# guodashun/peg-in-hole-gym

Measured on AMD Instinct MI355X. Metric: env-steps/sec, higher is better.
Workload: dtype f32

## Files before the change

### peg_in_hole_gym_amd/csrc/pih_common.h

```cpp
#pragma once
#include <string.h>
#include "../../include/pih.h"
#include "../../include/pih_model.h"
#include "pih_math.h"

namespace pih {

constexpr int NL = PIH_NL, ANL = PIH_ARM_NL, ONL = PIH_OBJ_NL, ND = PIH_NDOF;
constexpr int NSAMP = PIH_PIPE_NSAMP;
constexpr int CMAX = 48;
constexpr int CAMAX = 12;
constexpr int CL = 20;
constexpr int NROWC = 3 * CMAX;
constexpr int WPS = 39;
constexpr int WMS = 31;
constexpr int NMOT = 32;
constexpr int NLIM = 18;
static_assert(PIH_DBG_UDOT + ND <= PIH_DBG_NCONTACT && PIH_DBG_CONTACT + PIH_DBG_CONTACT_STRIDE * CMAX <= PIH_DBG_DINV &&
              PIH_DBG_DINV + 3 * CMAX <= PIH_DBG_CYCLES && PIH_DBG_XCC_ID < PIH_DEBUG_WORDS, "debug words of the peg-in-hole step (include/pih.h PIH_DBG_*) overlap");

PIH_CONST int L_PARENT[NL] = PIH_LINK_PARENT;
PIH_CONST int L_JTYPE[NL] = PIH_LINK_JTYPE;
PIH_CONST real L_RFIX[NL][9] = PIH_LINK_RFIX;
PIH_CONST real L_TFIX[NL][3] = PIH_LINK_TFIX;
// ... 422 lines not shown
    real tip[7]; tip_pose_serial(S, tip);
    Q4 tornq; tornq.x = tip[3]; tornq.y = tip[4]; tornq.z = tip[5]; tornq.w = tip[6];
    V3 rv = mul(q_to_m(tornq), mk(0, S[PIH_S_RANDY], 0));
    V3 tpos = mk(tip[0], tip[1], tip[2]) + rv;
    V3 tp = vel_constraint(eep, tpos, P.dv);
    if (st == 2 && st_prev != 2) o.grasp_angle = (real)atan2(rv.y, rv.x);
    if (st == 4 && st_prev != 4) o.attach_qz = tip[5];
    real yaw = yaw_from_quat(tornq);
    V3 hole = ld3(HOLE_POS);
    Q4 tq; tq.x = 0; tq.y = 0; tq.z = 0; tq.w = 1;
    int do_ik = 0;
    if (st == 1) { tp.z += (real)0.05; tq = quat_from_euler(0, -PIH_PI, PIH_PI / 2 + yaw); do_ik = 1; }
    else if (st == 2) { tp.z -= (real)0.01; tq = quat_from_euler(0, -PIH_PI, PIH_PI / 2 + yaw); do_ik = 1; }
    else if (st == 4) { tp = vel_constraint(eep, hole - mk((real)0.2, 0, 0), P.dv); tq = quat_from_euler(0, -PIH_PI, -PIH_PI); do_ik = 1; }
    else if (st == 5) { tp = vel_constraint(eep, hole - mk((real)0.04, 0, 0), P.dv); tq = quat_from_euler(0, -PIH_PI, -PIH_PI); do_ik = 1; }
    else if (st == 6) { tp = hole; tq = quat_from_euler(0, -PIH_PI, -PIH_PI); do_ik = 1; }
    else if (st == 8) { tp = mk((real)0.2, (real)-0.6, (real)0.4); tq = quat_from_euler(0, -PIH_PI, PIH_PI / 2); do_ik = 1; }
    if (do_ik) {
      real qs[7];
      ik_chain<PandaChain>(sw, ikT, P, q, tp, tq, qs);
#pragma unroll
      for (int i = 0; i < 7; i++) o.target[i] = qs[i];
    }
    const bool closed = st >= 3 && st < 7;
    const real ft = closed ? (real)0.006 : (real)0.02;
    o.target[7] = ft; o.target[8] = ft;
  }
  return o;
}
PIH_HD void controller_targets(real* S, const Params& P, const real* action) { const CtrlOut o = controller_compute(S, P, action); controller_apply(S, o); }

template <class W> PIH_HD void controller_rows(W& w, Shared& sh, const Params& P, int part = 0) {
  real* S = sh.S;
  int posctl_arm = 0; real kp_arm = 0, imp_arm = 1, kp_f = 0, imp_f = 1; int posctl_f = 0;
  if (P.mode == 0) {
    posctl_arm = posctl_f = 1; kp_arm = kp_f = 1; imp_arm = imp_f = (real)100000.0 * P.dt;
  } else {
    const int st = (int)S[PIH_S_FSM];
    if (st == 9) S[PIH_S_DONE] = 1;
    if (st >= 1) { posctl_arm = 1; kp_arm = (real)0.1; imp_arm = (real)(5.0 * 240.0) * P.dt; }
    const bool closed = st >= 3 && st < 7;
    posctl_f = 1; kp_f = (real)0.1; imp_f = (closed ? (real)20000 : (real)20) * P.dt;
  }
  w.par(NMOT, [&](int m) {
    if ((part == 1 && m < 9) || (part == 2 && m >= 9)) return;
    real vt = 0, imp = 1;
    if (m < 7) { if (posctl_arm) { vt = kp_arm * (S[PIH_S_TARGET + m] - S[PIH_S_QARM + m]) / P.dt; imp = imp_arm; } }
    else if (m < 9) { if (posctl_f) { vt = kp_f * (S[PIH_S_TARGET + m] - S[PIH_S_QARM + m]) / P.dt; imp = imp_f; } }
    sh.mrec[m][MR_RHS] = part == 2 ? (vt - sh.u[m]) * sh.mrec[m][MR_DINV] : vt;
    sh.mrec[m][MR_IMP] = imp;
  });
}

template <class W> PIH_HD void collide(W& w, Shared& sh, const Params& P) {
  const real r = (real)PIH_PIPE_RADIUS, margin = P.margin;
  w.par(NSAMP, [&](int i) {
    int L = ANL + SAMP_LINK[i];
    V3 p = ld3(sh.LO[L]) + mul(ldm(sh.a.LR[L]), mk(0, SAMP_Y[i], 0));
    st3(sh.a.SP[i], p);
  });
  auto emit = [&](int slot, int la, int lb, int key, V3 p, V3 n, real depth, real mu) {
    sh.c_la[slot] = la; sh.c_lb[slot] = lb; sh.c_key[slot] = key; st3(sh.c_p[slot], p); st3(sh.c_n[slot], n);
    sh.c_depth[slot] = depth; sh.c_mu[slot] = clampr(mu, -PIH_MAX_FRICTION, PIH_MAX_FRICTION);
  };
  w.alloc_reset(0);
  w.par_all(NSAMP, [&](int i, bool in) {
    bool valid = false; V3 sp = mk(0, 0, 0); real depth = 0; int L = 0;
    if (in && SAMP_VERTEX[i]) {
      sp = ld3(sh.a.SP[i]); depth = sp.z - (real)PIH_TABLE_Z - r; L = ANL + SAMP_LINK[i];
      valid = depth < margin;
    }
    int slot = w.alloc(valid);
    if (valid && slot < CMAX) {
      int vi = 0;
      { int s = SAMP_LINK[i]; vi = SAMP_Y[i] > (real)0.02 && s == 23 ? 24 : s; }
      emit(slot, L, -1, vi, mk(sp.x, sp.y, sp.z - r - (real)0.5 * depth), mk(0, 0, 1), depth, L_MU[L] * (real)PIH_TABLE_MU);
    }
  });
  const real hl = (real)PIH_HOLE_HALFLEN, rcx = (real)(0.5 * (PIH_HOLE_RIN + PIH_HOLE_ROUT)), hw = (real)(0.5 * (PIH_HOLE_ROUT - PIH_HOLE_RIN));
  w.par_all(NSAMP, [&](int i, bool in) {
    bool valid = false; V3 n = mk(0, 0, 0), p = mk(0, 0, 0); real depth = 0; int L = 0;
    if (in) {
      V3 sp = ld3(sh.a.SP[i]); V3 d = sp - ld3(HOLE_POS);
      real a = d.x, rho = (real)sqrt(d.y * d.y + d.z * d.z);
      real dx = absr(a) - hl, dy = absr(rho - rcx) - hw;
      if (!(dx > r + margin || dy > r + margin)) {
        real sa = a >= 0 ? (real)1 : (real)-1, sr = rho >= rcx ? (real)1 : (real)-1, ga, gr, sdf;
        if (dx <= 0 && dy <= 0) { if (dx > dy) { ga = sa; gr = 0; sdf = dx; } else { ga = 0; gr = sr; sdf = dy; } }
        else { real mx = dx > 0 ? dx : 0, my = dy > 0 ? dy : 0; sdf = (real)sqrt(mx * mx + my * my); ga = sa * mx / sdf; gr = sr * my / sdf; }
        depth = sdf - r;
        if (depth < margin && rho > (real)1e-9) {
          V3 rh = mk(0, d.y / rho, d.z / rho);
          n = mk(ga, gr * rh.y, gr * rh.z); p = sp - (r + (real)0.5 * depth) * n; L = ANL + SAMP_LINK[i]; valid = true;
        }
      }
    }
    int slot = w.alloc(valid);
    if (valid && slot < CMAX) emit(slot, L, -1, 100 + i, p, n, depth, L_MU[L] * (real)PIH_HOLE_MU);
  });
  int nca = 0;
  {
    const bool attached = P.mode == 1 && sh.S[PIH_S_FSM] >= 4 && sh.S[PIH_S_FSM] <= 6;
    const int before = w.alloc_count();
    w.par_all(1, [&](int i, bool in) {
      bool valid = in && i == 0 && attached;
      int slot = w.alloc(valid);
      if (valid && slot < CMAX) {
        int g = (int)sh.S[PIH_S_GRASP];
        int L = g == 0 ? ANL : NL - 1;
        V3 a1 = ld3(sh.LO[L]) + mul(ldm(sh.a.LR[L]), mk(0, (g == 0 ? (real)0.045 : (real)0.015) + sh.S[PIH_S_RANDY], 0));
        V3 ee; M3 eR; ee_pose(sh, ee, eR);
        V3 d = a1 - ee; real dist = norm(d);
        V3 n = dist > (real)1e-9 ? ((real)1 / dist) * d : mk(1, 0, 0);
        emit(slot, L, PIH_EE_PARENT, 2000, (real)0.5 * (a1 + ee), n, dist, (real)-1);
      }
    });
    w.par_all(1, [&](int i, bool in) {
      bool valid = in && i == 0 && attached && !P.attachball;
      int slot = w.alloc(valid);
      if (valid && slot < CMAX) {
        int g = (int)sh.S[PIH_S_GRASP];
        int L = g == 0 ? ANL : NL - 1;
        V3 ee; M3 eR; ee_pose(sh, ee, eR);
        const M3 Rcf = q_to_m(quat_from_euler(0, -PIH_PI, PIH_PI / 2 + sh.S[PIH_S_ATTACH_QZ]));
        const M3 Rc = mul(ldm(sh.a.LR[L]), Rcf);
        M3 eRt; for (int r = 0; r < 3; r++) for (int c = 0; c < 3; c++) eRt.m[3 * r + c] = eR.m[3 * c + r];
        const Q4 qe = m_to_q(mul(Rc, eRt));
        const V3 xyz = mk(qe.x, qe.y, qe.z);
        const real sn = norm(xyz); real ang = 2 * (real)atan2(sn, qe.w);
        if (ang > PIH_PI) ang -= 2 * PIH_PI;
        const V3 th = sn > (real)1e-12 ? (ang / sn) * xyz : mk(0, 0, 0);
        emit(slot, L, PIH_EE_PARENT, 2001, th, mk(1, 0, 0), 0, (real)-2);
      }
    });
    nca += w.alloc_count() - before;
  }
  if (P.armcol) w.par(PIH_ARM_NSPH, [&](int i) { const int L = ASPH_LINK[i]; st3(sh.a.ASP[i], ld3(sh.LO[L]) + mul(ldm(sh.a.LR[L]), ld3(ASPH_C[i]))); });
  if (P.armcol & 1) {
    const int before = w.alloc_count();
    const int allowed = CAMAX - nca;
    w.par_all(PIH_ARM_NSPH, [&](int i, bool in) {
      bool valid = false; V3 cw = mk(0, 0, 0); real depth = 0, rs = 0; int L = 0;
      if (in) {
        L = ASPH_LINK[i]; rs = ASPH_R[i];
        cw = ld3(sh.a.ASP[i]);
        depth = cw.z - (real)PIH_TABLE_Z - rs;
        valid = depth < margin;
      }
      int slot = w.alloc(valid);
      if (valid && slot < CMAX && (slot - before) < allowed) emit(slot, L, -1, 3000 + i, mk(cw.x, cw.y, cw.z - rs - (real)0.5 * depth), mk(0, 0, 1), depth, L_MU[L] * (real)PIH_TABLE_MU);
    });
    int used = w.alloc_count() - before;
    if (used > allowed) { used = allowed; w.alloc_reset(before + allowed); }
    nca += used;
  }
  const real padreach = norm(ld3(FBOX_H)) + r + margin + (real)1e-4;
  for (int f = 0; f < 2; f++) {
    const int LF = PIH_FINGER_LINK0 + f;
    M3 Rf = ldm(sh.a.LR[LF]); V3 bc = ld3(sh.LO[LF]) + mul(Rf, ld3(FBOX_C[f])); V3 bh = ld3(FBOX_H);
    const int before = w.alloc_count();
    const int allowed = CAMAX - nca;
    w.par_all(NSAMP, [&](int i, bool in) {
      bool valid = false; V3 n = mk(0, 0, 0), p = mk(0, 0, 0); real depth = 0; int L = 0;
      if (in) {
        V3 sp = ld3(sh.a.SP[i]); V3 d = sp - bc;
        if (dot(d, d) <= padreach * padreach) {
          V3 pl = tmul(Rf, d);
          V3 q = mk(clampr(pl.x, -bh.x, bh.x), clampr(pl.y, -bh.y, bh.y), clampr(pl.z, -bh.z, bh.z));
          bool inside = q.x == pl.x && q.y == pl.y && q.z == pl.z;
          V3 nl; real sdf;
          if (inside) {
            real bx = bh.x - absr(pl.x), by = bh.y - absr(pl.y), bz = bh.z - absr(pl.z);
            int ax = 0; real best = bx;
            if (by < best) { best = by; ax = 1; }
            if (bz < best) { best = bz; ax = 2; }
            nl = mk(ax == 0 ? (pl.x >= 0 ? (real)1 : (real)-1) : 0, ax == 1 ? (pl.y >= 0 ? (real)1 : (real)-1) : 0, ax == 2 ? (pl.z >= 0 ? (real)1 : (real)-1) : 0);
            sdf = -best;
          } else { V3 df = pl - q; sdf = norm(df); nl = ((real)1 / sdf) * df; }
          depth = sdf - r;
          if (depth < margin) { n = mul(Rf, nl); p = sp - (r + (real)0.5 * depth) * n; L = ANL + SAMP_LINK[i]; valid = true; }
        }
      }
      int slot = w.alloc(valid);
      if (valid && slot < CMAX && (slot - before) < allowed) emit(slot, L, LF, 300 + f * NSAMP + i, p, n, depth, L_MU[L] * L_MU[LF]);
    });
    int used = w.alloc_count() - before;
    if (used > allowed) { used = allowed; w.alloc_reset(before + allowed); }
    nca += used;
  }
  if (P.armcol & 2) {
    const int before = w.alloc_count();
    const int allowed = CAMAX - nca;
    w.par_all(NSAMP, [&](int i, bool in) {
      bool valid = false; V3 n = mk(0, 0, 0), p = mk(0, 0, 0); real depth = margin; int L = 0, bs = 0;
      if (in) {
        const V3 sp = ld3(sh.a.SP[i]);
#pragma unroll
        for (int s = PIH_ARM_PIPE_SPH0; s < PIH_ARM_NSPH; s++) {
          const V3 d = sp - ld3(sh.a.ASP[s]);
          const real d2 = dot(d, d), reach = margin + r + ASPH_R[s];
          if (d2 < reach * reach) {
            const real dist = (real)sqrt(d2), dep = dist - r - ASPH_R[s];
            if (dep < depth && dist > (real)1e-9) { depth = dep; bs = s; n = ((real)1 / dist) * d; valid = true; }
          }
        }
        if (valid) { p = sp - (r + (real)0.5 * depth) * n; L = ANL + SAMP_LINK[i]; }
      }
      int slot = w.alloc(valid);
      if (valid && slot < CMAX && (slot - before) < allowed) emit(slot, L, ASPH_LINK[bs], 5000 + bs * NSAMP + i, p, n, depth, L_MU[L] * L_MU[ASPH_LINK[bs]]);
    });
    int used = w.alloc_count() - before;
    if (used > allowed) { used = allowed; w.alloc_reset(before + allowed); }
    nca += used;
  }
  if (P.selfcol) {
    w.par_all(253, [&](int idx, bool in) {
      bool valid = false; V3 n = mk(0, 0, 0), p = mk(0, 0, 0); real depth = 0; int s = 0, t = 0;
      if (in) {
        s = (int)((real)0.5 * ((real)45 - (real)sqrt((real)(2025 - 8 * idx))));
        if ((s + 1) * (44 - s) / 2 <= idx) s++;
        if (s * (45 - s) / 2 > idx) s--;
        t = s + 2 + idx - s * (45 - s) / 2;
        auto vtx = [&](int v) -> V3 { int si = v == 0 ? 0 : (v == 24 ? NSAMP - 1 : 7 + 5 * (v - 1)); return ld3(sh.a.SP[si]); };
        V3 p1 = vtx(s), q1 = vtx(s + 1), p2 = vtx(t), q2 = vtx(t + 1);
        V3 dm = (p1 + q1) - (p2 + q2);
        V3 d1 = q1 - p1, d2 = q2 - p2;
        real a = dot(d1, d1), e = dot(d2, d2);
        const real reach = (real)sqrt(a) + (real)sqrt(e) + 2 * (2 * r + margin) + (real)1e-4;
        if (dot(dm, dm) <= reach * reach) {
          V3 rr = p1 - p2;
          real f = dot(d2, rr), ss, tt;
          const real EPS = (real)1e-12;
          if (a <= EPS && e <= EPS) { ss = tt = 0; }
          else if (a <= EPS) { ss = 0; tt = clampr(f / e, 0, 1); }
          else {
            real c = dot(d1, rr);
            if (e <= EPS) { tt = 0; ss = clampr(-c / a, 0, 1); }
            else {
              real b = dot(d1, d2), den = a * e - b * b;
              ss = den > EPS ? clampr((b * f - c * e) / den, 0, 1) : (real)0;
              tt = (b * ss + f) / e;
              if (tt < 0) { tt = 0; ss = clampr(-c / a, 0, 1); } else if (tt > 1) { tt = 1; ss = clampr((b - c) / a, 0, 1); }
            }
          }
          V3 c1 = p1 + ss * d1, c2 = p2 + tt * d2, d = c1 - c2;
          real dist = norm(d); depth = dist - 2 * r;
          if (depth < margin && dist >= (real)1e-9) { n = ((real)1 / dist) * d; p = (real)0.5 * (c1 + c2); valid = true; }
        }
      }
      int slot = w.alloc(valid);
      if (valid && slot < CMAX) emit(slot, ANL + s, ANL + t, 1000 + s * 24 + t, p, n, depth, L_MU[ANL + s] * L_MU[ANL + t]);
    });
  }
  int nc = w.alloc_count(); if (nc > CMAX) nc = CMAX;
  sh.nc = nc; sh.nca = nca;
}

PIH_HD void aba_root_inverse(Shared& sh, const real* Mx, areal* rootp) {
  areal Mq[6][6], Iv[6][6];
  for (int i = 0; i < 6; i++) for (int j = 0; j < 6; j++) { Mq[i][j] = Mx[8 * i + j]; Iv[i][j] = i == j ? (areal)1 : (areal)0; }
#pragma unroll
  for (int k = 0; k < 6; k++) {
    areal pv = (areal)1 / Mq[k][k];
#pragma unroll
    for (int j = 0; j < 6; j++) { Mq[k][j] *= pv; Iv[k][j] *= pv; }
#pragma unroll
    for (int i = 0; i < 6; i++) if (i != k) {
      areal f = Mq[i][k];
#pragma unroll
      for (int j = 0; j < 6; j++) { Mq[i][j] -= f * Mq[k][j]; Iv[i][j] -= f * Iv[k][j]; }
    }
  }
  for (int i = 0; i < 6; i++) { for (int j = 0; j < 6; j++) sh.Inv6[6 * i + j] = (real)Iv[i][j]; rootp[i] = Mx[8 * i + 6]; }
}
PIH_HD int aba_own_word(int i, int j) {
  const int ii = i < 3 ? i : i - 3, jj = j < 3 ? j : j - 3;
  const int sym = ii == jj ? ii : ii + jj + 2;
  if (i >= 6 || j >= 7) return 27;
  if (j == 6) return 21 + i;
  if (i < 3 && j < 3) return sym;
  if (i >= 3 && j >= 3) return 15 + sym;
  if (i < 3) return 6 + 3 * i + jj;
  return 6 + 3 * j + ii;
}
static_assert(NROWC >= 144, "scratch of the inward sweep aliases r_lam");

struct RowOut { real* wa; real* wp; };
PIH_HD real response(const Shared& sh, int la, int lb, V3 p, V3 dir, int jm, RowOut out, V3* dvp_out = nullptr, bool ang = false) {
  real jw = 0; V3 dvp = mk(0, 0, 0);
  bool arm = (la >= 0 && la < ANL) || (lb >= 0 && lb < ANL) || (jm >= 0 && jm < ANL);
  bool obj = (la >= ANL) || (lb >= ANL) || (jm >= ANL);
  if (arm && out.wa) {
    const bool aa_ = la >= 0 && la < ANL, ab_ = lb >= 0 && lb < ANL;
    const V3 rA = p - ld3(sh.LO[aa_ ? la : 0]), rB = p - ld3(sh.LO[ab_ ? lb : 0]);
    const V3 tqa = ang ? dir : cross(rA, dir), tqb = ang ? dir : cross(rB, dir), tl = ang ? mk(0, 0, 0) : dir;
    struct LinkC { V3 a, Ua, Ul, r; real Di; };
    auto linkc = [&](int L) __attribute__((always_inline)) -> LinkC {
      LinkC c; c.a = ld3(sh.LA[L]); c.Ua = ld3(sh.AU[L]); c.Ul = ld3(sh.AU[L] + 3); c.r = ld3(sh.AR[L]); c.Di = sh.ADinv[L]; return c;
    };
    V3 Qa[ANL], Ql[ANL]; real uu[ANL];
#pragma unroll
    for (int L = 0; L < ANL; L++) { Qa[L] = mk(0, 0, 0); Ql[L] = mk(0, 0, 0); }
    LinkC nx = linkc(ANL - 1);
#pragma unroll
    for (int L = ANL - 1; L >= 0; L--) {
      const LinkC c = nx;
// ... 204 lines not shown
```

### peg_in_hole_gym_amd/csrc/pih_wave.h

```cpp
#pragma once
#include <type_traits>
#include "pih_common.h"
#include "pih_mailbox.h"

namespace pih {

PIH_HD void debug_store_time(real* dbg, int at, long long t) { dbg[at] = (real)(t & 0xFFFF); dbg[at + 1] = (real)((t >> 16) & 0xFFFF); dbg[at + 2] = (real)((t >> 32) & 0xFFFF); }
PIH_HD void debug_store_hw_id(real* dbg) { dbg[PIH_DBG_HW_ID] = (real)(__builtin_amdgcn_s_getreg((15 << 11) | 4) & 0xFFFF); dbg[PIH_DBG_XCC_ID] = (real)__builtin_amdgcn_s_getreg((3 << 11) | 20); }

struct Wave {
  int l;
  int counter;
  static constexpr bool controller_inline = false;
  real* dbg = nullptr; int dbgmode = 0; long long t0 = 0, t1 = 0;
  PIH_HD void stamp(int k) { if (dbg && dbgmode == 2) { long long t = __builtin_readcyclecounter(); if (l == 0) dbg[PIH_DBG_CYCLES + k] = (real)(t - t0); t0 = t; } }
  PIH_HD void trace(int at, long long t) { if (l != 0) return; debug_store_time(dbg, at, t); if (at == PIH_DBG_T_START) debug_store_hw_id(dbg); }
  PIH_HD void phase_begin() { if (dbg && dbgmode == 2) { t1 = __builtin_readcyclecounter(); trace(PIH_DBG_T_START, (long long)__builtin_amdgcn_s_memrealtime()); } }
  PIH_HD void phase(int k) { if (dbg && dbgmode == 2) { long long t = __builtin_readcyclecounter(); if (l == 0) dbg[PIH_DBG_CYCLES + k] = (real)(t - t1); t1 = t; if (k == 7) trace(PIH_DBG_T_END, (long long)__builtin_amdgcn_s_memrealtime()); } }
  PIH_HD int lane() const { return l; }
  bool prio_on = true;
  PIH_HD void priority(int contacts) {
    if (!prio_on) return;
    if (contacts > 20) __builtin_amdgcn_s_setprio(3);
    else if (contacts > 14) __builtin_amdgcn_s_setprio(2);
// ... 103 lines not shown
#pragma unroll
  for (int off = 1; off < 32; off <<= 1) {
    const int src = vidx - off;
    const int sb = lane_byte((active && src >= cs) ? src : 63);
    M3 Rs; V3 os;
#pragma unroll
    for (int k = 0; k < 9; k++) Rs.m[k] = from_lane(R.m[k], sb);
    os = mk(from_lane(o.x, sb), from_lane(o.y, sb), from_lane(o.z, sb));
    o = os + mul(Rs, o); R = mul(Rs, R);
  }
  if (active) {
    stm(sh.a.LR[L], R); st3(sh.LO[L], o);
    st3(sh.LA[L], mul(R, ld3(L_AXIS[L])));
    st3(sh.a.LRC[L], mul(R, ld3(L_COM[L])));
    sts3(sh.a.LIC[L], rot_sym(R, lds3(L_INERTIA[L])));
  }
  w.sync();
}
PIH_HD V3 from_lane3(V3 v, int byte_addr) { return mk(from_lane(v.x, byte_addr), from_lane(v.y, byte_addr), from_lane(v.z, byte_addr)); }
PIH_HD V3 chain_prefix_sum(V3 t, int lane, int chain_start) {
  V3 acc = t;
#pragma unroll
  for (int off = 1; off < 32; off <<= 1) {
    const int src = lane - off;
    const V3 o = from_lane3(acc, 4 * (src < 0 ? 0 : src));
    if (src >= chain_start) acc = acc + o;
  }
  return acc;
}
PIH_HD void link_velocities_scan(Shared& sh, int lane) {
  const bool active = lane < NL;
  const int L = active ? lane : NL - 1;
  const int jt = L == ANL ? PIH_JT_FLOATING : ((L == ANL - 1 || L == ANL - 2) ? PIH_JT_PRISMATIC : PIH_JT_REVOLUTE);
  const int par = (L == 0 || L == ANL) ? -1 : (L == ANL - 1 ? ANL - 3 : L - 1);
  const int cs = L < ANL ? 0 : ANL, d = link_dof(L);
  const V3 aq = sh.u[d] * ld3(sh.LA[L]);
  const V3 tw = jt == PIH_JT_FLOATING ? ld3(&sh.u[d + 3]) : (jt == PIH_JT_REVOLUTE ? aq : mk(0, 0, 0));
  V3 wv = chain_prefix_sum(tw, lane, cs);
  const V3 tw7 = from_lane3(tw, 4 * (ANL - 2));
  if (L == ANL - 1) wv = wv - tw7;
  const V3 wp = from_lane3(wv, 4 * (par < 0 ? 0 : par));
  V3 tv;
  if (jt == PIH_JT_FLOATING) tv = ld3(&sh.u[d]);
  else {
    tv = jt == PIH_JT_PRISMATIC ? aq : mk(0, 0, 0);
    if (par >= 0) tv = tv + cross(wp, ld3(sh.LO[L]) - ld3(sh.LO[par]));
  }
  V3 vv = chain_prefix_sum(tv, lane, cs);
  const V3 tv7 = from_lane3(tv, 4 * (ANL - 2));
  if (L == ANL - 1) vv = vv - tv7;
  if (active) { st3(sh.VW[L], wv); st3(sh.VV[L], vv); }
}
PIH_HD void link_velocities(Wave& w, Shared& sh) { w.sync(); link_velocities_scan(sh, w.lane()); w.sync(); }

PIH_HD void aba_inward(Wave& w, Shared& sh, areal* rootp) {
  real* const Mx = sh.r_lam;
  {
    const int l = w.lane(), i = l >> 3, j = l & 7;
    const int ia = i < 3 ? i : (i < 6 ? i - 3 : 0), ja = j < 3 ? j : (j < 6 ? j - 3 : 0);
    const int i1 = ia == 2 ? 0 : ia + 1, i2 = ia == 0 ? 2 : ia - 1, j1 = ja == 2 ? 0 : ja + 1, j2 = ja == 0 ? 2 : ja - 1;
    const bool typeA = i < 3 && j < 3, typeB = i < 3 && j >= 3 && j < 6, typeBt = i >= 3 && i < 6 && j < 3, typeP = i < 3 && j == 6;
    const int own_off = aba_own_word(i, j);
    int kA = 0, kB = 0, s1 = l, s2 = l;
    if (typeA) { kA = i1; kB = i2; s1 = 8 * j + 3 + i2; s2 = 8 * j + 3 + i1; }
    else if (typeB) { kA = i1; kB = i2; s1 = 8 * (3 + i2) + j; s2 = 8 * (3 + i1) + j; }
    else if (typeBt) { kA = j1; kB = j2; s1 = 8 * (3 + j2) + i; s2 = 8 * (3 + j1) + i; }
    else if (typeP) { kA = i1; kB = i2; s1 = 8 * (3 + i2) + 6; s2 = 8 * (3 + i1) + 6; }
    const real m1 = (typeA || typeB || typeBt || typeP) ? (real)1 : (real)0, m2 = typeA ? (real)1 : (real)0;
    int s3 = l, s4 = l, s5 = l, s6 = l, s7 = l, s8 = l;
    if (typeA) { s3 = 8 * i + 3 + j1; s4 = 8 * (3 + i2) + 3 + j1; s5 = 8 * (3 + i1) + 3 + j1; s6 = 8 * i + 3 + j2; s7 = 8 * (3 + i2) + 3 + j2; s8 = 8 * (3 + i1) + 3 + j2; }
    const int sUj = j < 6 ? 8 * j : l;
    auto link = [&](int L, real m, bool up) __attribute__((always_inline)) -> real {
      const int jt = joint_type(L);
      const int sb = jt == PIH_JT_REVOLUTE ? 0 : 3;
      const V3 a = ld3(sh.LA[L]);
      const real rA = m1 * sh.AR[L][kA], rB = m1 * sh.AR[L][kB], rG = m2 * sh.AR[L][j2], rK = m2 * sh.AR[L][j1];
      const real cj = j < 6 ? sh.a.CB[L][j] : (real)0;
      const int js = j - sb;
      const real sj = js == 0 ? a.x : (js == 1 ? a.y : (js == 2 ? a.z : (real)0));
      const real Ui = sum8(m * sj);
      const real Uj = from_lane(Ui, 4 * sUj);
      const real D = a.x * rdlane(Ui, 8 * sb) + a.y * rdlane(Ui, 8 * (sb + 1)) + a.z * rdlane(Ui, 8 * (sb + 2));
      const real tau = 0;
      const real u = tau - (a.x * rdlane(m, 8 * sb + 6) + a.y * rdlane(m, 8 * (sb + 1) + 6) + a.z * rdlane(m, 8 * (sb + 2) + 6));
      const real Di = (real)1 / D;
      if (j == 0 && i < 6) sh.AU[L][i] = Ui;
      if (l == 0) { sh.ADinv[L] = Di; sh.Au[L] = u; }
      if (!up) return 0;
      real ma = j < 6 ? m - Ui * Uj * Di : m;
      const real s = sum8(j < 6 ? ma * cj : (real)0);
      if (j == 6) ma = m + s + Ui * (u * Di);
      const real X1 = from_lane(ma, 4 * s1), X2 = from_lane(ma, 4 * s2), X3 = from_lane(ma, 4 * s3), X4 = from_lane(ma, 4 * s4),
                 X5 = from_lane(ma, 4 * s5), X6 = from_lane(ma, 4 * s6), X7 = from_lane(ma, 4 * s7), X8 = from_lane(ma, 4 * s8);
      return ma + rA * X1 - rB * X2 - ((X3 + rA * X4 - rB * X5) * rG - (X6 + rA * X7 - rB * X8) * rK);
    };
    real carry_p = 0, carry_a = 0, hold = 0;
#pragma nounroll
    for (int k = 0; k < 8; k++) {
      const int Lp = NL - 1 - k, La = ANL - 1 - k;
      const real own_p = sh.a.IAP[Lp][own_off], own_a = sh.a.IAP[La][own_off];
      const real mp = k == 0 ? own_p : own_p + carry_p;
      const real ma = k < 2 ? own_a : own_a + carry_a;
      const real vp = link(Lp, mp, true), va = link(La, ma, true);
      carry_p = vp;
      if (k == 0) hold = va;
      else if (k == 1) carry_a = va + hold;
// ... 714 lines not shown
```

Before: 11.99 million.

## Fuse collision narrow-phase into a single-wave pass with register-held candidates

Adds a Wave-specialised collide that computes every sample's table, tube, finger-pad and arm-sphere candidates in one pass, keeping sample points and arm-sphere centres in registers instead of re-reading shared memory per test and synchronising between separate parallel loops. Per-link friction and sphere constants are resolved from constexpr tables by select chains, and inline asm pins keep values in vector or scalar registers. Contact slots are still allocated in the original order so the emitted contacts stay identical. It raises register pressure because many candidates are live at once, which could lower occupancy.

```diff
diff --git a/peg_in_hole_gym_amd/csrc/pih_common.h b/peg_in_hole_gym_amd/csrc/pih_common.h
--- a/peg_in_hole_gym_amd/csrc/pih_common.h
+++ b/peg_in_hole_gym_amd/csrc/pih_common.h
@@ -498,52 +498,159 @@
   });
 }
 
+struct Cand { bool valid; V3 p, n; real depth; };
+PIH_HD Cand no_cand(real depth = 0) { Cand c; c.valid = false; c.p = mk(0, 0, 0); c.n = mk(0, 0, 0); c.depth = depth; return c; }
+PIH_HD V3 sample_point(const Shared& sh, int L, real y) { return ld3(sh.LO[L]) + mul(ldm(sh.a.LR[L]), mk(0, y, 0)); }
+PIH_HD int vertex_key(int slink, real sy) { return sy > (real)0.02 && slink == 23 ? 24 : slink; }
+PIH_HD void emit_contact(Shared& sh, int slot, int la, int lb, int key, V3 p, V3 n, real depth, real mu) {
+  sh.c_la[slot] = la; sh.c_lb[slot] = lb; sh.c_key[slot] = key; st3(sh.c_p[slot], p); st3(sh.c_n[slot], n);
+  sh.c_depth[slot] = depth; sh.c_mu[slot] = clampr(mu, -PIH_MAX_FRICTION, PIH_MAX_FRICTION);
+}
+PIH_HD Cand sphere_vs_table(V3 c, real rs, real margin) {
+  Cand o; o.depth = c.z - (real)PIH_TABLE_Z - rs; o.valid = o.depth < margin;
+  o.p = mk(c.x, c.y, c.z - rs - (real)0.5 * o.depth); o.n = mk(0, 0, 1);
+  return o;
+}
+PIH_HD Cand sample_vs_tube(V3 sp, V3 hole, real r, real margin) {
+  const real hl = (real)PIH_HOLE_HALFLEN, rcx = (real)(0.5 * (PIH_HOLE_RIN + PIH_HOLE_ROUT)), hw = (real)(0.5 * (PIH_HOLE_ROUT - PIH_HOLE_RIN));
+  Cand o = no_cand();
+  V3 d = sp - hole;
+  real a = d.x, rho = (real)sqrt(d.y * d.y + d.z * d.z);
+  real dx = absr(a) - hl, dy = absr(rho - rcx) - hw;
+  if (!(dx > r + margin || dy > r + margin)) {
+    real sa = a >= 0 ? (real)1 : (real)-1, sr = rho >= rcx ? (real)1 : (real)-1, ga, gr, sdf;
+    if (dx <= 0 && dy <= 0) { if (dx > dy) { ga = sa; gr = 0; sdf = dx; } else { ga = 0; gr = sr; sdf = dy; } }
+    else { real mx = dx > 0 ? dx : 0, my = dy > 0 ? dy : 0; sdf = (real)sqrt(mx * mx + my * my); ga = sa * mx / sdf; gr = sr * my / sdf; }
+    o.depth = sdf - r;
+    if (o.depth < margin && rho > (real)1e-9) {
+      V3 rh = mk(0, d.y / rho, d.z / rho);
+      o.n = mk(ga, gr * rh.y, gr * rh.z); o.p = sp - (r + (real)0.5 * o.depth) * o.n; o.valid = true;
+    }
+  }
+  return o;
+}
+PIH_HD real pad_reach(V3 bh, real r, real margin) { return norm(bh) + r + margin + (real)1e-4; }
+PIH_HD Cand sample_vs_pad(V3 sp, const M3& Rf, V3 bc, V3 bh, real padreach, real r, real margin) {
+  Cand o = no_cand();
+  V3 d = sp - bc;
+  if (dot(d, d) <= padreach * padreach) {
+    V3 pl = tmul(Rf, d);
+    V3 q = mk(clampr(pl.x, -bh.x, bh.x), clampr(pl.y, -bh.y, bh.y), clampr(pl.z, -bh.z, bh.z));
+    bool inside = q.x == pl.x && q.y == pl.y && q.z == pl.z;
+    V3 nl; real sdf;
+    if (inside) {
+      real bx = bh.x - absr(pl.x), by = bh.y - absr(pl.y), bz = bh.z - absr(pl.z);
+      int ax = 0; real best = bx;
+      if (by < best) { best = by; ax = 1; }
+      if (bz < best) { best = bz; ax = 2; }
+      nl = mk(ax == 0 ? (pl.x >= 0 ? (real)1 : (real)-1) : 0, ax == 1 ? (pl.y >= 0 ? (real)1 : (real)-1) : 0, ax == 2 ? (pl.z >= 0 ? (real)1 : (real)-1) : 0);
+      sdf = -best;
+    } else { V3 df = pl - q; sdf = norm(df); nl = ((real)1 / sdf) * df; }
+    o.depth = sdf - r;
+    if (o.depth < margin) { o.n = mul(Rf, nl); o.p = sp - (r + (real)0.5 * o.depth) * o.n; o.valid = true; }
+  }
+  return o;
+}
+template <class FC, class FR> PIH_HD Cand sample_vs_arm_spheres(V3 sp, FC centre, FR radius, real r, real margin, int& bs) {
+  Cand o = no_cand(margin);
+  bs = 0;
+#pragma unroll
+  for (int s = PIH_ARM_PIPE_SPH0; s < PIH_ARM_NSPH; s++) {
+    const V3 d = sp - centre(s);
+    const real d2 = dot(d, d), reach = margin + r + radius(s);
+    if (d2 < reach * reach) {
+      const real dist = (real)sqrt(d2), dep = dist - r - radius(s);
+      if (dep < o.depth && dist > (real)1e-9) { o.depth = dep; bs = s; o.n = ((real)1 / dist) * d; o.valid = true; }
+    }
+  }
+  if (o.valid) o.p = sp - (r + (real)0.5 * o.depth) * o.n;
+  return o;
+}
+PIH_HD void pair_of_index(int idx, int& s, int& t) {
+  s = (int)((real)0.5 * ((real)45 - (real)sqrt((real)(2025 - 8 * idx))));
+  if ((s + 1) * (44 - s) / 2 <= idx) s++;
+  if (s * (45 - s) / 2 > idx) s--;
+  t = s + 2 + idx - s * (45 - s) / 2;
+}
+PIH_HD int vertex_sample(int v) { return v == 0 ? 0 : (v == 24 ? NSAMP - 1 : 7 + 5 * (v - 1)); }
+PIH_HD Cand segment_pair(V3 p1, V3 q1, V3 p2, V3 q2, real r, real margin) {
+  Cand o = no_cand();
+  V3 dm = (p1 + q1) - (p2 + q2);
+  V3 d1 = q1 - p1, d2 = q2 - p2;
+  real a = dot(d1, d1), e = dot(d2, d2);
+  const real reach = (real)sqrt(a) + (real)sqrt(e) + 2 * (2 * r + margin) + (real)1e-4;
+  if (dot(dm, dm) <= reach * reach) {
+    V3 rr = p1 - p2;
+    real f = dot(d2, rr), ss, tt;
+    const real EPS = (real)1e-12;
+    if (a <= EPS && e <= EPS) { ss = tt = 0; }
+    else if (a <= EPS) { ss = 0; tt = clampr(f / e, 0, 1); }
+    else {
+      real c = dot(d1, rr);
+      if (e <= EPS) { tt = 0; ss = clampr(-c / a, 0, 1); }
+      else {
+        real b = dot(d1, d2), den = a * e - b * b;
+        ss = den > EPS ? clampr((b * f - c * e) / den, 0, 1) : (real)0;
+        tt = (b * ss + f) / e;
+        if (tt < 0) { tt = 0; ss = clampr(-c / a, 0, 1); } else if (tt > 1) { tt = 1; ss = clampr((b - c) / a, 0, 1); }
+      }
+    }
+    V3 c1 = p1 + ss * d1, c2 = p2 + tt * d2, d = c1 - c2;
+    real dist = norm(d); o.depth = dist - 2 * r;
+    if (o.depth < margin && dist >= (real)1e-9) { o.n = ((real)1 / dist) * d; o.p = (real)0.5 * (c1 + c2); o.valid = true; }
+  }
+  return o;
+}
+PIH_HD Cand attach_ball_contact(Shared& sh, int& L) {
+  Cand o;
+  int g = (int)sh.S[PIH_S_GRASP];
+  L = g == 0 ? ANL : NL - 1;
+  V3 a1 = ld3(sh.LO[L]) + mul(ldm(sh.a.LR[L]), mk(0, (g == 0 ? (real)0.045 : (real)0.015) + sh.S[PIH_S_RANDY], 0));
+  V3 ee; M3 eR; ee_pose(sh, ee, eR);
+  V3 d = a1 - ee; real dist = norm(d);
+  o.n = dist > (real)1e-9 ? ((real)1 / dist) * d : mk(1, 0, 0);
+  o.p = (real)0.5 * (a1 + ee); o.depth = dist; o.valid = true;
+  return o;
+}
+PIH_HD Cand attach_weld_contact(Shared& sh, int& L) {
+  Cand o;
+  int g = (int)sh.S[PIH_S_GRASP];
+  L = g == 0 ? ANL : NL - 1;
+  V3 ee; M3 eR; ee_pose(sh, ee, eR);
+  const M3 Rcf = q_to_m(quat_from_euler(0, -PIH_PI, PIH_PI / 2 + sh.S[PIH_S_ATTACH_QZ]));
+  const M3 Rc = mul(ldm(sh.a.LR[L]), Rcf);
+  M3 eRt; for (int r = 0; r < 3; r++) for (int c = 0; c < 3; c++) eRt.m[3 * r + c] = eR.m[3 * c + r];
+  const Q4 qe = m_to_q(mul(Rc, eRt));
+  const V3 xyz = mk(qe.x, qe.y, qe.z);
+  const real sn = norm(xyz); real ang = 2 * (real)atan2(sn, qe.w);
+  if (ang > PIH_PI) ang -= 2 * PIH_PI;
+  o.p = sn > (real)1e-12 ? (ang / sn) * xyz : mk(0, 0, 0);
+  o.n = mk(1, 0, 0); o.depth = 0; o.valid = true;
+  return o;
+}
+
 template <class W> PIH_HD void collide(W& w, Shared& sh, const Params& P) {
   const real r = (real)PIH_PIPE_RADIUS, margin = P.margin;
-  w.par(NSAMP, [&](int i) {
-    int L = ANL + SAMP_LINK[i];
-    V3 p = ld3(sh.LO[L]) + mul(ldm(sh.a.LR[L]), mk(0, SAMP_Y[i], 0));
-    st3(sh.a.SP[i], p);
-  });
-  auto emit = [&](int slot, int la, int lb, int key, V3 p, V3 n, real depth, real mu) {
-    sh.c_la[slot] = la; sh.c_lb[slot] = lb; sh.c_key[slot] = key; st3(sh.c_p[slot], p); st3(sh.c_n[slot], n);
-    sh.c_depth[slot] = depth; sh.c_mu[slot] = clampr(mu, -PIH_MAX_FRICTION, PIH_MAX_FRICTION);
-  };
+  w.stamp(16);
+  w.par(NSAMP, [&](int i) { st3(sh.a.SP[i], sample_point(sh, ANL + SAMP_LINK[i], SAMP_Y[i])); });
+  auto emit = [&](int slot, int la, int lb, int key, V3 p, V3 n, real depth, real mu) { emit_contact(sh, slot, la, lb, key, p, n, depth, mu); };
   w.alloc_reset(0);
   w.par_all(NSAMP, [&](int i, bool in) {
-    bool valid = false; V3 sp = mk(0, 0, 0); real depth = 0; int L = 0;
-    if (in && SAMP_VERTEX[i]) {
-      sp = ld3(sh.a.SP[i]); depth = sp.z - (real)PIH_TABLE_Z - r; L = ANL + SAMP_LINK[i];
-      valid = depth < margin;
-    }
-    int slot = w.alloc(valid);
-    if (valid && slot < CMAX) {
-      int vi = 0;
-      { int s = SAMP_LINK[i]; vi = SAMP_Y[i] > (real)0.02 && s == 23 ? 24 : s; }
-      emit(slot, L, -1, vi, mk(sp.x, sp.y, sp.z - r - (real)0.5 * depth), mk(0, 0, 1), depth, L_MU[L] * (real)PIH_TABLE_MU);
+    Cand c = no_cand();
+    if (in && SAMP_VERTEX[i]) c = sphere_vs_table(ld3(sh.a.SP[i]), r, margin);
+    int slot = w.alloc(c.valid);
+    if (c.valid && slot < CMAX) {
+      const int L = ANL + SAMP_LINK[i];
+      emit(slot, L, -1, vertex_key(SAMP_LINK[i], SAMP_Y[i]), c.p, c.n, c.depth, L_MU[L] * (real)PIH_TABLE_MU);
     }
   });
-  const real hl = (real)PIH_HOLE_HALFLEN, rcx = (real)(0.5 * (PIH_HOLE_RIN + PIH_HOLE_ROUT)), hw = (real)(0.5 * (PIH_HOLE_ROUT - PIH_HOLE_RIN));
   w.par_all(NSAMP, [&](int i, bool in) {
-    bool valid = false; V3 n = mk(0, 0, 0), p = mk(0, 0, 0); real depth = 0; int L = 0;
-    if (in) {
-      V3 sp = ld3(sh.a.SP[i]); V3 d = sp - ld3(HOLE_POS);
-      real a = d.x, rho = (real)sqrt(d.y * d.y + d.z * d.z);
-      real dx = absr(a) - hl, dy = absr(rho - rcx) - hw;
-      if (!(dx > r + margin || dy > r + margin)) {
-        real sa = a >= 0 ? (real)1 : (real)-1, sr = rho >= rcx ? (real)1 : (real)-1, ga, gr, sdf;
-        if (dx <= 0 && dy <= 0) { if (dx > dy) { ga = sa; gr = 0; sdf = dx; } else { ga = 0; gr = sr; sdf = dy; } }
-        else { real mx = dx > 0 ? dx : 0, my = dy > 0 ? dy : 0; sdf = (real)sqrt(mx * mx + my * my); ga = sa * mx / sdf; gr = sr * my / sdf; }
-        depth = sdf - r;
-        if (depth < margin && rho > (real)1e-9) {
-          V3 rh = mk(0, d.y / rho, d.z / rho);
-          n = mk(ga, gr * rh.y, gr * rh.z); p = sp - (r + (real)0.5 * depth) * n; L = ANL + SAMP_LINK[i]; valid = true;
-        }
-      }
-    }
-    int slot = w.alloc(valid);
-    if (valid && slot < CMAX) emit(slot, L, -1, 100 + i, p, n, depth, L_MU[L] * (real)PIH_HOLE_MU);
+    Cand c = no_cand();
+    if (in) c = sample_vs_tube(ld3(sh.a.SP[i]), ld3(HOLE_POS), r, margin);
+    int slot = w.alloc(c.valid);
+    if (c.valid && slot < CMAX) { const int L = ANL + SAMP_LINK[i]; emit(slot, L, -1, 100 + i, c.p, c.n, c.depth, L_MU[L] * (real)PIH_HOLE_MU); }
   });
+  w.stamp(17);
   int nca = 0;
   {
     const bool attached = P.mode == 1 && sh.S[PIH_S_FSM] >= 4 && sh.S[PIH_S_FSM] <= 6;
@@ -551,33 +658,12 @@
     w.par_all(1, [&](int i, bool in) {
       bool valid = in && i == 0 && attached;
       int slot = w.alloc(valid);
-      if (valid && slot < CMAX) {
-        int g = (int)sh.S[PIH_S_GRASP];
-        int L = g == 0 ? ANL : NL - 1;
-        V3 a1 = ld3(sh.LO[L]) + mul(ldm(sh.a.LR[L]), mk(0, (g == 0 ? (real)0.045 : (real)0.015) + sh.S[PIH_S_RANDY], 0));
-        V3 ee; M3 eR; ee_pose(sh, ee, eR);
-        V3 d = a1 - ee; real dist = norm(d);
-        V3 n = dist > (real)1e-9 ? ((real)1 / dist) * d : mk(1, 0, 0);
-        emit(slot, L, PIH_EE_PARENT, 2000, (real)0.5 * (a1 + ee), n, dist, (real)-1);
-      }
+      if (valid && slot < CMAX) { int L; const Cand c = attach_ball_contact(sh, L); emit(slot, L, PIH_EE_PARENT, 2000, c.p, c.n, c.depth, (real)-1); }
     });
     w.par_all(1, [&](int i, bool in) {
       bool valid = in && i == 0 && attached && !P.attachball;
       int slot = w.alloc(valid);
-      if (valid && slot < CMAX) {
-        int g = (int)sh.S[PIH_S_GRASP];
-        int L = g == 0 ? ANL : NL - 1;
-        V3 ee; M3 eR; ee_pose(sh, ee, eR);
-        const M3 Rcf = q_to_m(quat_from_euler(0, -PIH_PI, PIH_PI / 2 + sh.S[PIH_S_ATTACH_QZ]));
-        const M3 Rc = mul(ldm(sh.a.LR[L]), Rcf);
-        M3 eRt; for (int r = 0; r < 3; r++) for (int c = 0; c < 3; c++) eRt.m[3 * r + c] = eR.m[3 * c + r];
-        const Q4 qe = m_to_q(mul(Rc, eRt));
-        const V3 xyz = mk(qe.x, qe.y, qe.z);
-        const real sn = norm(xyz); real ang = 2 * (real)atan2(sn, qe.w);
-        if (ang > PIH_PI) ang -= 2 * PIH_PI;
-        const V3 th = sn > (real)1e-12 ? (ang / sn) * xyz : mk(0, 0, 0);
-        emit(slot, L, PIH_EE_PARENT, 2001, th, mk(1, 0, 0), 0, (real)-2);
-      }
+      if (valid && slot < CMAX) { int L; const Cand c = attach_weld_contact(sh, L); emit(slot, L, PIH_EE_PARENT, 2001, c.p, c.n, c.depth, (real)-2); }
     });
     nca += w.alloc_count() - before;
   }
@@ -586,118 +672,63 @@
     const int before = w.alloc_count();
     const int allowed = CAMAX - nca;
     w.par_all(PIH_ARM_NSPH, [&](int i, bool in) {
-      bool valid = false; V3 cw = mk(0, 0, 0); real depth = 0, rs = 0; int L = 0;
-      if (in) {
-        L = ASPH_LINK[i]; rs = ASPH_R[i];
-        cw = ld3(sh.a.ASP[i]);
-        depth = cw.z - (real)PIH_TABLE_Z - rs;
-        valid = depth < margin;
-      }
-      int slot = w.alloc(valid);
-      if (valid && slot < CMAX && (slot - before) < allowed) emit(slot, L, -1, 3000 + i, mk(cw.x, cw.y, cw.z - rs - (real)0.5 * depth), mk(0, 0, 1), depth, L_MU[L] * (real)PIH_TABLE_MU);
+      Cand c = no_cand();
+      if (in) c = sphere_vs_table(ld3(sh.a.ASP[i]), ASPH_R[i], margin);
+      int slot = w.alloc(c.valid);
+      if (c.valid && slot < CMAX && (slot - before) < allowed) { const int L = ASPH_LINK[i]; emit(slot, L, -1, 3000 + i, c.p, c.n, c.depth, L_MU[L] * (real)PIH_TABLE_MU); }
     });
     int used = w.alloc_count() - before;
     if (used > allowed) { used = allowed; w.alloc_reset(before + allowed); }
     nca += used;
   }
-  const real padreach = norm(ld3(FBOX_H)) + r + margin + (real)1e-4;
+  w.stamp(18);
+  const real padreach = pad_reach(ld3(FBOX_H), r, margin);
   for (int f = 0; f < 2; f++) {
     const int LF = PIH_FINGER_LINK0 + f;
     M3 Rf = ldm(sh.a.LR[LF]); V3 bc = ld3(sh.LO[LF]) + mul(Rf, ld3(FBOX_C[f])); V3 bh = ld3(FBOX_H);
     const int before = w.alloc_count();
     const int allowed = CAMAX - nca;
     w.par_all(NSAMP, [&](int i, bool in) {
-      bool valid = false; V3 n = mk(0, 0, 0), p = mk(0, 0, 0); real depth = 0; int L = 0;
-      if (in) {
-        V3 sp = ld3(sh.a.SP[i]); V3 d = sp - bc;
-        if (dot(d, d) <= padreach * padreach) {
-          V3 pl = tmul(Rf, d);
-          V3 q = mk(clampr(pl.x, -bh.x, bh.x), clampr(pl.y, -bh.y, bh.y), clampr(pl.z, -bh.z, bh.z));
-          bool inside = q.x == pl.x && q.y == pl.y && q.z == pl.z;
-          V3 nl; real sdf;
-          if (inside) {
-            real bx = bh.x - absr(pl.x), by = bh.y - absr(pl.y), bz = bh.z - absr(pl.z);
-            int ax = 0; real best = bx;
-            if (by < best) { best = by; ax = 1; }
-            if (bz < best) { best = bz; ax = 2; }
-            nl = mk(ax == 0 ? (pl.x >= 0 ? (real)1 : (real)-1) : 0, ax == 1 ? (pl.y >= 0 ? (real)1 : (real)-1) : 0, ax == 2 ? (pl.z >= 0 ? (real)1 : (real)-1) : 0);
-            sdf = -best;
-          } else { V3 df = pl - q; sdf = norm(df); nl = ((real)1 / sdf) * df; }
-          depth = sdf - r;
-          if (depth < margin) { n = mul(Rf, nl); p = sp - (r + (real)0.5 * depth) * n; L = ANL + SAMP_LINK[i]; valid = true; }
-        }
-      }
-      int slot = w.alloc(valid);
-      if (valid && slot < CMAX && (slot - before) < allowed) emit(slot, L, LF, 300 + f * NSAMP + i, p, n, depth, L_MU[L] * L_MU[LF]);
+      Cand c = no_cand();
+      if (in) c = sample_vs_pad(ld3(sh.a.SP[i]), Rf, bc, bh, padreach, r, margin);
+      int slot = w.alloc(c.valid);
+      if (c.valid && slot < CMAX && (slot - before) < allowed) { const int L = ANL + SAMP_LINK[i]; emit(slot, L, LF, 300 + f * NSAMP + i, c.p, c.n, c.depth, L_MU[L] * L_MU[LF]); }
     });
     int used = w.alloc_count() - before;
     if (used > allowed) { used = allowed; w.alloc_reset(before + allowed); }
     nca += used;
   }
+  w.stamp(19);
   if (P.armcol & 2) {
     const int before = w.alloc_count();
     const int allowed = CAMAX - nca;
     w.par_all(NSAMP, [&](int i, bool in) {
-      bool valid = false; V3 n = mk(0, 0, 0), p = mk(0, 0, 0); real depth = margin; int L = 0, bs = 0;
-      if (in) {
-        const V3 sp = ld3(sh.a.SP[i]);
-#pragma unroll
-        for (int s = PIH_ARM_PIPE_SPH0; s < PIH_ARM_NSPH; s++) {
-          const V3 d = sp - ld3(sh.a.ASP[s]);
-          const real d2 = dot(d, d), reach = margin + r + ASPH_R[s];
-          if (d2 < reach * reach) {
-            const real dist = (real)sqrt(d2), dep = dist - r - ASPH_R[s];
-            if (dep < depth && dist > (real)1e-9) { depth = dep; bs = s; n = ((real)1 / dist) * d; valid = true; }
-          }
-        }
-        if (valid) { p = sp - (r + (real)0.5 * depth) * n; L = ANL + SAMP_LINK[i]; }
+      Cand c = no_cand(); int bs = 0;
+      if (in) c = sample_vs_arm_spheres(ld3(sh.a.SP[i]), [&](int s) { return ld3(sh.a.ASP[s]); }, [&](int s) { return ASPH_R[s]; }, r, margin, bs);
+      int slot = w.alloc(c.valid);
+      if (c.valid && slot < CMAX && (slot - before) < allowed) {
+        const int L = ANL + SAMP_LINK[i];
+        emit(slot, L, ASPH_LINK[bs], 5000 + bs * NSAMP + i, c.p, c.n, c.depth, L_MU[L] * L_MU[ASPH_LINK[bs]]);
       }
-      int slot = w.alloc(valid);
-      if (valid && slot < CMAX && (slot - before) < allowed) emit(slot, L, ASPH_LINK[bs], 5000 + bs * NSAMP + i, p, n, depth, L_MU[L] * L_MU[ASPH_LINK[bs]]);
     });
     int used = w.alloc_count() - before;
     if (used > allowed) { used = allowed; w.alloc_reset(before + allowed); }
     nca += used;
   }
+  w.stamp(20);
   if (P.selfcol) {
     w.par_all(253, [&](int idx, bool in) {
-      bool valid = false; V3 n = mk(0, 0, 0), p = mk(0, 0, 0); real depth = 0; int s = 0, t = 0;
+      Cand c = no_cand(); int s = 0, t = 0;
       if (in) {
-        s = (int)((real)0.5 * ((real)45 - (real)sqrt((real)(2025 - 8 * idx))));
-        if ((s + 1) * (44 - s) / 2 <= idx) s++;
-        if (s * (45 - s) / 2 > idx) s--;
-        t = s + 2 + idx - s * (45 - s) / 2;
-        auto vtx = [&](int v) -> V3 { int si = v == 0 ? 0 : (v == 24 ? NSAMP - 1 : 7 + 5 * (v - 1)); return ld3(sh.a.SP[si]); };
-        V3 p1 = vtx(s), q1 = vtx(s + 1), p2 = vtx(t), q2 = vtx(t + 1);
-        V3 dm = (p1 + q1) - (p2 + q2);
-        V3 d1 = q1 - p1, d2 = q2 - p2;
-        real a = dot(d1, d1), e = dot(d2, d2);
-        const real reach = (real)sqrt(a) + (real)sqrt(e) + 2 * (2 * r + margin) + (real)1e-4;
-        if (dot(dm, dm) <= reach * reach) {
-          V3 rr = p1 - p2;
-          real f = dot(d2, rr), ss, tt;
-          const real EPS = (real)1e-12;
-          if (a <= EPS && e <= EPS) { ss = tt = 0; }
-          else if (a <= EPS) { ss = 0; tt = clampr(f / e, 0, 1); }
-          else {
-            real c = dot(d1, rr);
-            if (e <= EPS) { tt = 0; ss = clampr(-c / a, 0, 1); }
-            else {
-              real b = dot(d1, d2), den = a * e - b * b;
-              ss = den > EPS ? clampr((b * f - c * e) / den, 0, 1) : (real)0;
-              tt = (b * ss + f) / e;
-              if (tt < 0) { tt = 0; ss = clampr(-c / a, 0, 1); } else if (tt > 1) { tt = 1; ss = clampr((b - c) / a, 0, 1); }
-            }
-          }
-          V3 c1 = p1 + ss * d1, c2 = p2 + tt * d2, d = c1 - c2;
-          real dist = norm(d); depth = dist - 2 * r;
-          if (depth < margin && dist >= (real)1e-9) { n = ((real)1 / dist) * d; p = (real)0.5 * (c1 + c2); valid = true; }
-        }
+        pair_of_index(idx, s, t);
+        auto vtx = [&](int v) -> V3 { return ld3(sh.a.SP[vertex_sample(v)]); };
+        c = segment_pair(vtx(s), vtx(s + 1), vtx(t), vtx(t + 1), r, margin);
       }
-      int slot = w.alloc(valid);
-      if (valid && slot < CMAX) emit(slot, ANL + s, ANL + t, 1000 + s * 24 + t, p, n, depth, L_MU[ANL + s] * L_MU[ANL + t]);
+      int slot = w.alloc(c.valid);
+      if (c.valid && slot < CMAX) emit(slot, ANL + s, ANL + t, 1000 + s * 24 + t, c.p, c.n, c.depth, L_MU[ANL + s] * L_MU[ANL + t]);
     });
   }
+  w.stamp(21);
   int nc = w.alloc_count(); if (nc > CMAX) nc = CMAX;
   sh.nc = nc; sh.nca = nca;
 }
diff --git a/peg_in_hole_gym_amd/csrc/pih_wave.h b/peg_in_hole_gym_amd/csrc/pih_wave.h
--- a/peg_in_hole_gym_amd/csrc/pih_wave.h
+++ b/peg_in_hole_gym_amd/csrc/pih_wave.h
@@ -179,6 +179,183 @@
   if (active) { st3(sh.VW[L], wv); st3(sh.VV[L], vv); }
 }
 PIH_HD void link_velocities(Wave& w, Shared& sh) { w.sync(); link_velocities_scan(sh, w.lane()); w.sync(); }
+
+constexpr double K_LMU[NL] = PIH_LINK_MU;
+constexpr int K_ASPH_LINK[PIH_ARM_NSPH] = PIH_ARM_SPH_LINK;
+constexpr double K_ASPH_R[PIH_ARM_NSPH] = PIH_ARM_SPH_R;
+constexpr double K_FBOX_C[2][3] = PIH_FINGER_BOX_C;
+constexpr double K_FBOX_H[3] = PIH_FINGER_BOX_H;
+constexpr double K_HOLE_POS[3] = PIH_HOLE_POS;
+template <int L0, int N> PIH_HD real link_mu(int k) {
+  real mu = (real)K_LMU[L0 + N / 2];
+#pragma unroll
+  for (int j = 0; j < N; j++) if (K_LMU[L0 + j] != K_LMU[L0 + N / 2]) mu = k == j ? (real)K_LMU[L0 + j] : mu;
+  return mu;
+}
+PIH_HD real pipe_link_mu(int s) { return link_mu<ANL, ONL>(s); }
+PIH_HD void arm_sphere_link(int s, int& link, real& mu) {
+  link = K_ASPH_LINK[0]; mu = (real)K_LMU[K_ASPH_LINK[0]];
+#pragma unroll
+  for (int j = 1; j < PIH_ARM_NSPH; j++) { link = s == j ? K_ASPH_LINK[j] : link; mu = s == j ? (real)K_LMU[K_ASPH_LINK[j]] : mu; }
+}
+PIH_HD void pin(V3& v) { __asm__ volatile("" : "+v"(v.x), "+v"(v.y), "+v"(v.z)); }
+PIH_HD Cand arm_sphere_vs_table(V3 c, real rs, real margin) {
+  Cand o;
+  real k = -(real)PIH_TABLE_Z - rs; __asm__ volatile("" : "+v"(k));
+  o.depth = c.z + k; o.valid = o.depth < margin;
+  real t = rs + (real)0.5 * o.depth; __asm__ volatile("" : "+v"(t));
+  o.p = mk(c.x, c.y, c.z - t); o.n = mk(0, 0, 1);
+  return o;
+}
+PIH_HD real arm_sphere_radius(int s) { real v = (real)K_ASPH_R[s]; __asm__ volatile("" : "+s"(v)); return v; }
+PIH_HD void collide(Wave& w, Shared& sh, const Params& P) {
+  const real r = (real)PIH_PIPE_RADIUS, margin = P.margin;
+  const int lane = w.lane();
+  w.stamp(16);
+  bool inr[2]; int sidx[2], slink[2], svert[2]; real sy[2];
+#pragma unroll
+  for (int c = 0; c < 2; c++) {
+    sidx[c] = lane + 64 * c; inr[c] = sidx[c] < NSAMP;
+    const int j = inr[c] ? sidx[c] : NSAMP - 1;
+    slink[c] = SAMP_LINK[j]; sy[c] = SAMP_Y[j]; svert[c] = SAMP_VERTEX[j];
+  }
+  const bool isph = lane < PIH_ARM_NSPH;
+  const int jsph = isph ? lane : 0;
+  const int alink = ASPH_LINK[jsph]; const real arad = ASPH_R[jsph]; const V3 acen = ld3(ASPH_C[jsph]);
+  w.sync();
+  V3 sp[2];
+#pragma unroll
+  for (int c = 0; c < 2; c++) {
+    sp[c] = sample_point(sh, ANL + slink[c], sy[c]);
+    if (inr[c]) st3(sh.a.SP[sidx[c]], sp[c]);
+    pin(sp[c]);
+  }
+  V3 cw = mk(0, 0, 0);
+  if (P.armcol) {
+    cw = ld3(sh.LO[alink]) + mul(ldm(sh.a.LR[alink]), acen);
+    if (isph) st3(sh.a.ASP[lane], cw);
+    pin(cw);
+  }
+  w.sync();
+  const V3 hole = mk((real)K_HOLE_POS[0], (real)K_HOLE_POS[1], (real)K_HOLE_POS[2]);
+  const V3 bh = mk((real)K_FBOX_H[0], (real)K_FBOX_H[1], (real)K_FBOX_H[2]);
+  const real padreach = pad_reach(bh, r, margin);
+  M3 Rf[2]; V3 bc[2];
+#pragma unroll
+  for (int f = 0; f < 2; f++) {
+    Rf[f] = ldm(sh.a.LR[PIH_FINGER_LINK0 + f]);
+    bc[f] = ld3(sh.LO[PIH_FINGER_LINK0 + f]) + mul(Rf[f], mk((real)K_FBOX_C[f][0], (real)K_FBOX_C[f][1], (real)K_FBOX_C[f][2]));
+  }
+  const bool armpipe = (P.armcol & 2) != 0;
+  V3 ac[PIH_ARM_NSPH]; real ar[PIH_ARM_NSPH];
+#pragma unroll
+  for (int s = 0; s < PIH_ARM_NSPH; s++) { ac[s] = armpipe && s >= PIH_ARM_PIPE_SPH0 ? ld3(sh.a.ASP[s]) : mk(0, 0, 0); ar[s] = arm_sphere_radius(s); }
+  Cand ct[2], ch[2], cp[2][2], ca[2]; int bs[2];
+#pragma unroll
+  for (int c = 0; c < 2; c++) {
+    ct[c] = no_cand(); ch[c] = no_cand(); cp[0][c] = no_cand(); cp[1][c] = no_cand(); ca[c] = no_cand(); bs[c] = 0;
+    if (inr[c] && svert[c]) ct[c] = sphere_vs_table(sp[c], r, margin);
+    if (inr[c]) ch[c] = sample_vs_tube(sp[c], hole, r, margin);
+    if (inr[c]) cp[0][c] = sample_vs_pad(sp[c], Rf[0], bc[0], bh, padreach, r, margin);
+    if (inr[c]) cp[1][c] = sample_vs_pad(sp[c], Rf[1], bc[1], bh, padreach, r, margin);
+    if (armpipe && inr[c]) ca[c] = sample_vs_arm_spheres(sp[c], [&](int s) { return ac[s]; }, [&](int s) { return ar[s]; }, r, margin, bs[c]);
+  }
+  w.stamp(17);
+  w.alloc_reset(0);
+#pragma unroll
+  for (int c = 0; c < 2; c++) {
+    const int slot = w.alloc(ct[c].valid);
+    if (ct[c].valid && slot < CMAX)
+      emit_contact(sh, slot, ANL + slink[c], -1, vertex_key(slink[c], sy[c]), ct[c].p, ct[c].n, ct[c].depth, pipe_link_mu(slink[c]) * (real)PIH_TABLE_MU);
+  }
+#pragma unroll
+  for (int c = 0; c < 2; c++) {
+    const int slot = w.alloc(ch[c].valid);
+    if (ch[c].valid && slot < CMAX) emit_contact(sh, slot, ANL + slink[c], -1, 100 + sidx[c], ch[c].p, ch[c].n, ch[c].depth, pipe_link_mu(slink[c]) * (real)PIH_HOLE_MU);
+  }
+  int nca = 0;
+  {
+    const bool attached = P.mode == 1 && sh.S[PIH_S_FSM] >= 4 && sh.S[PIH_S_FSM] <= 6;
+    const int before = w.alloc_count();
+    {
+      const bool valid = lane == 0 && attached;
+      const int slot = w.alloc(valid);
+      if (valid && slot < CMAX) { int L; const Cand c = attach_ball_contact(sh, L); emit_contact(sh, slot, L, PIH_EE_PARENT, 2000, c.p, c.n, c.depth, (real)-1); }
+    }
+    {
+      const bool valid = lane == 0 && attached && !P.attachball;
+      const int slot = w.alloc(valid);
+      if (valid && slot < CMAX) { int L; const Cand c = attach_weld_contact(sh, L); emit_contact(sh, slot, L, PIH_EE_PARENT, 2001, c.p, c.n, c.depth, (real)-2); }
+    }
+    nca += w.alloc_count() - before;
+  }
+  if (P.armcol & 1) {
+    const int before = w.alloc_count();
+    const int allowed = CAMAX - nca;
+    Cand c = no_cand();
+    if (isph) c = arm_sphere_vs_table(cw, arad, margin);
+    const int slot = w.alloc(c.valid);
+    if (c.valid && slot < CMAX && (slot - before) < allowed) {
+      int L; real mu; arm_sphere_link(lane, L, mu);
+      emit_contact(sh, slot, L, -1, 3000 + lane, c.p, c.n, c.depth, mu * (real)PIH_TABLE_MU);
+    }
+    int used = w.alloc_count() - before;
+    if (used > allowed) { used = allowed; w.alloc_reset(before + allowed); }
+    nca += used;
+  }
+  w.stamp(18);
+#pragma unroll
+  for (int f = 0; f < 2; f++) {
+    const int LF = PIH_FINGER_LINK0 + f;
+    const int before = w.alloc_count();
+    const int allowed = CAMAX - nca;
+#pragma unroll
+    for (int c = 0; c < 2; c++) {
+      const Cand& k = cp[f][c];
+      const int slot = w.alloc(k.valid);
+      if (k.valid && slot < CMAX && (slot - before) < allowed)
+        emit_contact(sh, slot, ANL + slink[c], LF, 300 + f * NSAMP + sidx[c], k.p, k.n, k.depth, pipe_link_mu(slink[c]) * (real)K_LMU[LF]);
+    }
+    int used = w.alloc_count() - before;
+    if (used > allowed) { used = allowed; w.alloc_reset(before + allowed); }
+    nca += used;
+  }
+  w.stamp(19);
+  if (armpipe) {
+    const int before = w.alloc_count();
+    const int allowed = CAMAX - nca;
+#pragma unroll
+    for (int c = 0; c < 2; c++) {
+      const int slot = w.alloc(ca[c].valid);
+      if (ca[c].valid && slot < CMAX && (slot - before) < allowed) {
+        int lb; real mub; arm_sphere_link(bs[c], lb, mub);
+        emit_contact(sh, slot, ANL + slink[c], lb, 5000 + bs[c] * NSAMP + sidx[c], ca[c].p, ca[c].n, ca[c].depth, pipe_link_mu(slink[c]) * mub);
+      }
+    }
+    int used = w.alloc_count() - before;
+    if (used > allowed) { used = allowed; w.alloc_reset(before + allowed); }
+    nca += used;
+  }
+  w.stamp(20);
+  if (P.selfcol) {
+#pragma unroll
+    for (int b = 0; b < 253; b += 64) {
+      const int idx = b + lane;
+      Cand c = no_cand(); int s = 0, t = 0;
+      if (idx < 253) {
+        pair_of_index(idx, s, t);
+        auto vtx = [&](int v) -> V3 { return ld3(sh.a.SP[vertex_sample(v)]); };
+        c = segment_pair(vtx(s), vtx(s + 1), vtx(t), vtx(t + 1), r, margin);
+      }
+      const int slot = w.alloc(c.valid);
+      if (c.valid && slot < CMAX) emit_contact(sh, slot, ANL + s, ANL + t, 1000 + s * 24 + t, c.p, c.n, c.depth, pipe_link_mu(s) * pipe_link_mu(t));
+    }
+  }
+  w.stamp(21);
+  int nc = w.alloc_count(); if (nc > CMAX) nc = CMAX;
+  sh.nc = nc; sh.nca = nca;
+  w.sync();
+}
 
 PIH_HD void aba_inward(Wave& w, Shared& sh, areal* rootp) {
   real* const Mx = sh.r_lam;
```

Result: faster. 12.12 million, median of 6 (+1.0%).
